# Linux-cpp-lisp/navigation-by-deja-vu

Measured on AMD Instinct MI355X. Metric: view-comparisons/sec (sensor x library x headings), higher is better.
Workload: dtype u8

## Files before the change

### navigation-by-deja-vu_amd/csrc/dejavu_hip.hip

```cpp
#include "dejavu_kernels.h"
#include "../../include/dejavu.h"

#include <algorithm>
#include <atomic>
#include <chrono>
#include <cmath>
#include <limits>
#include <cstdarg>
#include <cstddef>
#include <cstdint>
#include <cstdio>
#include <cstdlib>
#include <cstring>
#include <new>
#include <string>
#include <vector>

using namespace dv;

static_assert(sizeof(StepResultDev) == sizeof(dv_step_result) + sizeof(unsigned long long) &&
              offsetof(StepResultDev, check) == sizeof(dv_step_result), "device record = host record + check word");
static_assert(kMaxHeadings == DV_MAX_HEADINGS && kMaxHues == DV_MAX_HUE_PLANES, "header constants differ");
static_assert(kResSenseError == DV_RES_SENSE_ERROR, "header constants differ");

// ... 77 lines not shown
    uint4* d_tiles = nullptr;
    size_t tile_bytes = 0;

    unsigned char* d_raw_patches = nullptr;
    unsigned* d_prep = nullptr;
    PrepAcc* d_acc = nullptr;
    int acc_parity = 0;
    PrepBits pbits{};
    unsigned* d_one = nullptr;
    unsigned long long* d_bsum2 = nullptr;
    unsigned long long* d_bsum = nullptr;
    unsigned long long* d_ctmp = nullptr;
    int int_has_hs = 0, int_has_v = 0;
    int finish_vb_env = 0;
    int fenced_env = -1;
    int finish_fused = 1;
    unsigned* d_part = nullptr;
    unsigned long long* d_pmax = nullptr;
    int n_partial = 0;
    int nchunk = 1;
    int nchunk_cap = 1;
    int target_items = 0;
    int waves_per_cu = 0;
    int shape_env = 0;
    int force_shape = 0;
    int tuned_shape[4] = {0, 0, 0, 0};
    float tuned_us[4][6] = {};
    bool bits_ok = false;
    bool mixed = false;
    bool hs_bytes_pass = false;
    BitCfg bcfg{};
    uint4* d_btiles = nullptr;
    size_t btile_bytes = 0;
    uint4* d_coef = nullptr;
    bool coef_ready = false;
    bool prep_dwords_ready = false;
    int bits_env = 1;
    int mfma_tiles_env = 0, mfma_chunk_env = 0;
    const int* int_hsconst = nullptr;
    const int* int_vconst = nullptr;
    bool fuse_request = false;
    bool epilogue_fused = false;
    bool fp4_ok = false;
    int fp4_env = 1;
    uint4* d_coef4 = nullptr;
    uint4* d_ctiles = nullptr;
    size_t ctile_bytes = 0;
    int vcode_env = 0;
    int last_form = 0;
    int fuse_env = 1;
    int lc_env = 1;
    int ht_env = 2;
    int ring_env = 0;
    int mixed_env = 1;
    int tune_all_env = 0;
    int fail_alloc_env = 0;
    int lib_allocs = 0;
    int fused_nb = 0;
    int group_pad_kb = -1;
    int allow_signed = 1;
    double* d_fam = nullptr;
    double* d_scene = nullptr;
    StepState* d_state = nullptr;
    unsigned long long* d_cand = nullptr;
    double* d_cand_exact = nullptr;
    int result_slot = 0;
    struct PassSet {
        unsigned char* raw = nullptr; uint4* coef = nullptr; uint4* coef4 = nullptr; PrepAcc* acc = nullptr; int parity = 0;
        unsigned long long* bsum = nullptr; unsigned long long* ctmp = nullptr; StepState* state = nullptr;
        unsigned long long* cand = nullptr; double* cand_exact = nullptr;
        bool coef_ready = false, prep_dwords_ready = false, patches_sensed = false;
        int A = 0, APAD = 0, n_agents = 1, A_agent = 0, fused_nb = 0;
    };
    static constexpr int kExtraSets = 8;
    PassSet extra[kExtraSets];
    int n_extra = 0;
    int cur_set = 0;
    hipStream_t batch_stream = nullptr;
    hipStream_t batch_stream3 = nullptr;
    hipEvent_t ev_a = nullptr, ev_b = nullptr;
    bool defer_fold = false;
    int deferred_force = 0, deferred_seq = 0;
    int lc22_env = 1;
    int chain_order_env = -1;
    int chains_env = 2;
    StepResultDev* h_result = nullptr;
    StepResultDev* d_result = nullptr;
    double* d_record = nullptr;
    unsigned long long* d_keys = nullptr;
    double* h_scene = nullptr;
    int A = 0, APAD = 0;
    int n_agents = 1, A_agent = 0;
    bool step_pending = false;
    bool patches_sensed = false;
    int seq = 0;
    double* h_mbox = nullptr;
    double* d_mbox = nullptr;
    int mbox_rank = 0, mbox_world = 0, mbox_slots = 0;
    double* h_pub = nullptr;
    double* d_pub = nullptr;
    int64_t pub_cap = 0;
    unsigned long long pub_seq = 0;
    int spin_wait = 1;
    bool last_want_scene = false;
    double delta = 0.0;
    double wr_lo = 1.0, wr_hi = 0.0;
    AgentW* d_wts = nullptr;
    AgentW* h_wts = nullptr;
    int h_wts_cap = 0;
    bool wts_on = false;

    unsigned char* d_land = nullptr;
    SensorCfg sensor{};
    bool have_sensor = false;
    unsigned char* d_lut = nullptr;
    Pose* d_poses = nullptr;
    size_t poses_cap = 0;
    unsigned char* d_sense = nullptr;
    size_t sense_cap = 0;
    unsigned long long* d_sense_err = nullptr;
    std::vector<Pose> h_poses;

    double* d_path = nullptr;
    int64_t n_path = 0;
    unsigned char* d_cover = nullptr;
    unsigned char* d_cover_slots = nullptr;
    int n_cover_slots = 0;
    unsigned long long* d_minkeys = nullptr;
    unsigned long long* h_minkeys = nullptr;
    PathErrState* d_errstate = nullptr;
    PathErrOut* h_errout = nullptr;
    PathErrOut* d_errout = nullptr;
    unsigned long long err_enq = 0, err_deq = 0;
    int agent_pending = 0;
    bool err_on_main = false;

    hipEvent_t t0 = nullptr, t1 = nullptr;
    int profile = 0;
    long long profile_count = 0;
    std::vector<hipEvent_t> pev;
    size_t pev_used = 0;
};

static int fail(dv_ctx* c, int code, const char* fmt, ...) {
    char buf[512];
    va_list ap;
    va_start(ap, fmt);
    vsnprintf(buf, sizeof buf, fmt, ap);
    va_end(ap);
    if (c) c->err = buf; else g_create_error = buf;
    return code;
}

#define HIP_TRY(ctx, expr)                                                                      \
    do {                                                                                        \
        hipError_t e_ = (expr);                                                                 \
        if (e_ != hipSuccess)                                                                   \
            return fail(ctx, e_ == hipErrorOutOfMemory ? DV_ERR_OOM : DV_ERR_HIP, "%s: %s (%s:%d)", #expr, \
                        hipGetErrorString(e_), __FILE__, __LINE__);                             \
    } while (0)

static void use_set(dv_ctx* c, int which);
static void free_library(dv_ctx* c) {
    auto F = [](auto*& p) { if (p) { (void)hipFree(p); p = nullptr; } };
    use_set(c, 0);
    for (int j = 0; j < dv_ctx::kExtraSets; ++j) {
        dv_ctx::PassSet& a = c->extra[j];
        F(a.raw); F(a.coef); F(a.coef4); F(a.acc); F(a.bsum); F(a.ctmp); F(a.state); F(a.cand); F(a.cand_exact);
        a = dv_ctx::PassSet{};
    }
    c->n_extra = 0;
    F(c->d_tiles); F(c->d_raw_patches); F(c->d_prep); F(c->d_acc); F(c->d_one); F(c->d_fam); F(c->d_scene);
    F(c->d_part); F(c->d_pmax); F(c->d_record); F(c->d_keys); F(c->d_bsum); F(c->d_bsum2); F(c->d_ctmp);
    F(c->d_ftiles); F(c->d_fraw); F(c->d_fprep); F(c->d_fpart); F(c->d_fprep4); F(c->d_fvnorm); F(c->d_fpnorm); F(c->d_flower); F(c->d_fprepb);
    F(c->d_u8tiles); F(c->d_u8raw); F(c->d_u8prep); F(c->d_u8part); F(c->d_vnorm); F(c->d_pnorm);
    F(c->d_btiles); F(c->d_coef); F(c->d_coef4); F(c->d_ctiles); c->ctile_bytes = 0;
    c->pbits = PrepBits{};
    c->bits_ok = false; c->coef_ready = false; c->btile_bytes = 0;
    c->metric = 0;
    F(c->d_state); F(c->d_cand); F(c->d_cand_exact);
    if (c->h_result) { (void)hipHostFree(c->h_result); c->h_result = nullptr; c->d_result = nullptr; }
    if (c->h_scene) { (void)hipHostFree(c->h_scene); c->h_scene = nullptr; }
    c->have_lib = false;
    for (int i = 0; i < 4; ++i) c->tuned_shape[i] = 0;
    c->A = 0;
    c->step_pending = false;
}

extern "C" const char* dv_version(void) { return "dejavu-mi355x 0.1 (gfx950)"; }

extern "C" const char* dv_last_error(const dv_ctx* ctx) { return ctx ? ctx->err.c_str() : g_create_error.c_str(); }

extern "C" int dv_create(dv_ctx** out, int device_id) {
    if (!out) return fail(nullptr, DV_ERR_INVALID, "dv_create: out is NULL");
    *out = nullptr;
    int n = 0;
    HIP_TRY(nullptr, hipGetDeviceCount(&n));
    if (device_id < 0 || device_id >= n) return fail(nullptr, DV_ERR_INVALID, "dv_create: device %d of %d", device_id, n);
    HIP_TRY(nullptr, hipSetDevice(device_id));
    dv_ctx* c = new (std::nothrow) dv_ctx();
    if (!c) return fail(nullptr, DV_ERR_OOM, "dv_create: out of host memory");
    c->device = device_id;
    hipError_t e = hipStreamCreateWithFlags(&c->own_stream, hipStreamNonBlocking);
    if (e == hipSuccess) e = hipStreamCreateWithFlags(&c->aux_stream, hipStreamNonBlocking);
    if (e == hipSuccess) e = hipEventCreate(&c->t0);
    if (e == hipSuccess) e = hipEventCreate(&c->t1);
    if (e != hipSuccess) {
        fail(nullptr, DV_ERR_HIP, "dv_create: %s", hipGetErrorString(e));
        delete c;
        return DV_ERR_HIP;
    }
    c->stream = c->own_stream;
    auto env_int = [](const char* name, int& dst, int lo, int hi) {
        if (const char* t = getenv(name)) { const int v = atoi(t); if (v >= lo && v <= hi) dst = v; }
    };
    env_int("DEJAVU_TARGET_ITEMS", c->target_items, 1, 1 << 24);
    env_int("DEJAVU_WPC", c->waves_per_cu, 1, 32);
    env_int("DEJAVU_SHAPE", c->shape_env, 0, 6);
    env_int("DEJAVU_BITS", c->bits_env, 0, 2);
    env_int("DEJAVU_MFMA_TILES", c->mfma_tiles_env, 0, 2);
    env_int("DEJAVU_MFMA_CHUNK", c->mfma_chunk_env, 0, 32);
    env_int("DEJAVU_FINISH", c->finish_fused, 0, 2);
    env_int("DEJAVU_FENCED", c->fenced_env, 0, 1);
    env_int("DEJAVU_FINISH_VB", c->finish_vb_env, 0, 16);
    env_int("DEJAVU_FUSE", c->fuse_env, 0, 1);
    env_int("DEJAVU_FP4", c->fp4_env, 0, 1);
    env_int("DEJAVU_VCODE", c->vcode_env, 0, 1);
    env_int("DEJAVU_SIGNED", c->allow_signed, 0, 1);
    env_int("DEJAVU_GPAD", c->group_pad_kb, 0, 4096);
    env_int("DEJAVU_SPIN", c->spin_wait, 0, 1);
    env_int("DEJAVU_LC", c->lc_env, 0, 2);
    env_int("DEJAVU_HT", c->ht_env, 1, 2);
    env_int("DEJAVU_RING", c->ring_env, 0, 2);
    env_int("DEJAVU_MIXED", c->mixed_env, 0, 1);
    env_int("DEJAVU_TUNE_ALL", c->tune_all_env, 0, 1);
    env_int("DEJAVU_SSD_MFMA", c->ssd_mfma_env, 0, 3);
    env_int("DEJAVU_CHAINS", c->chains_env, 1, 3);
    env_int("DEJAVU_CHAIN_ORDER", c->chain_order_env, -1, 2);
    env_int("DEJAVU_LC22", c->lc22_env, 0, 1);
    env_int("DEJAVU_NT", c->nt_env, 0, 1);
    env_int("DEJAVU_TEST_FAIL_ALLOC", c->fail_alloc_env, 0, 64);
    *out = c;
    return DV_OK;
}

extern "C" void dv_destroy(dv_ctx* c) {
    if (!c) return;
    (void)hipSetDevice(c->device);
    (void)hipStreamSynchronize(c->stream);
    free_library(c);
    if (c->d_land) (void)hipFree(c->d_land);
    if (c->d_lut) (void)hipFree(c->d_lut);
    if (c->d_poses) (void)hipFree(c->d_poses);
    if (c->d_sense) (void)hipFree(c->d_sense);
    if (c->d_sense_err) (void)hipFree(c->d_sense_err);
    if (c->d_path) (void)hipFree(c->d_path);
    if (c->d_cover) (void)hipFree(c->d_cover);
    if (c->d_cover_slots) (void)hipFree(c->d_cover_slots);
    if (c->d_minkeys) (void)hipFree(c->d_minkeys);
    if (c->h_minkeys) (void)hipHostFree(c->h_minkeys);
    if (c->d_errstate) (void)hipFree(c->d_errstate);
    if (c->h_errout) (void)hipHostFree(c->h_errout);
    if (c->h_pub) (void)hipHostFree(c->h_pub);
    if (c->h_mbox) (void)hipHostUnregister(c->h_mbox);
    for (auto e : c->pev) (void)hipEventDestroy(e);
    if (c->t0) (void)hipEventDestroy(c->t0);
    if (c->t1) (void)hipEventDestroy(c->t1);
    if (c->aux_stream) { (void)hipStreamSynchronize(c->aux_stream); (void)hipStreamDestroy(c->aux_stream); }
    if (c->batch_stream) { (void)hipStreamSynchronize(c->batch_stream); (void)hipStreamDestroy(c->batch_stream); }
    if (c->batch_stream3) { (void)hipStreamSynchronize(c->batch_stream3); (void)hipStreamDestroy(c->batch_stream3); }
    if (c->d_wts) (void)hipFree(c->d_wts);
    if (c->h_wts) (void)hipHostFree(c->h_wts);
    if (c->ev_a) (void)hipEventDestroy(c->ev_a);
    if (c->ev_b) (void)hipEventDestroy(c->ev_b);
    if (c->own_stream) (void)hipStreamDestroy(c->own_stream);
    delete c;
}

extern "C" int dv_set_stream(dv_ctx* c, void* s) {
    if (!c) return DV_ERR_INVALID;
    HIP_TRY(c, hipStreamSynchronize(c->stream));
    c->stream = s ? (hipStream_t)s : c->own_stream;
    return DV_OK;
}

extern "C" int dv_set_exact(dv_ctx* c, int exact) {
    if (!c) return DV_ERR_INVALID;
    c->exact = exact ? 1 : 0;
    return DV_OK;
}

extern "C" int dv_set_mailbox(dv_ctx* c, void* host_base, int64_t bytes, int rank, int world) {
    if (!c) return DV_ERR_INVALID;
    HIP_TRY(c, hipSetDevice(c->device));
    HIP_TRY(c, hipStreamSynchronize(c->stream));
    if (c->h_mbox) { (void)hipHostUnregister(c->h_mbox); c->h_mbox = nullptr; c->d_mbox = nullptr; }
    if (!host_base) return DV_OK;
    const int64_t per_slot = (int64_t)world * kMboxEntry * (int64_t)sizeof(double);
    if (world < 1 || world > 64 || rank < 0 || rank >= world || bytes < per_slot || ((uintptr_t)host_base & 4095))
        return fail(c, DV_ERR_INVALID, "dv_set_mailbox: bad arguments");
    HIP_TRY(c, hipHostRegister(host_base, (size_t)bytes, hipHostRegisterMapped | hipHostRegisterPortable));
    c->h_mbox = (double*)host_base;
    HIP_TRY(c, hipHostGetDevicePointer((void**)&c->d_mbox, host_base, 0));
    c->mbox_rank = rank; c->mbox_world = world; c->mbox_slots = (int)(bytes / per_slot);
    return DV_OK;
}

extern "C" int dv_mailbox_post(dv_ctx* c, int slot, uint64_t seq) {
    if (!c) return DV_ERR_INVALID;
    if (!c->d_mbox || slot < 0 || slot >= c->mbox_slots) return fail(c, DV_ERR_STATE, "dv_mailbox_post: no mailbox or bad slot");
    if (!c->have_lib || c->A < 1) return fail(c, DV_ERR_STATE, "no library or no resident patches");
    HIP_TRY(c, hipSetDevice(c->device));
    double* entry = c->d_mbox + ((size_t)slot * c->mbox_world + c->mbox_rank) * kMboxEntry;
    hipLaunchKernelGGL(k_post, dim3(1), dim3(256), 0, c->stream, c->d_record, entry, 3 + 4 * c->A, (unsigned long long)seq);
    HIP_TRY(c, hipGetLastError());
    return DV_OK;
}

extern "C" int dv_mailbox_wait(dv_ctx* c, int slot, uint64_t seq, uint64_t rank_mask, double* records, int64_t stride,
                               int timeout_ms) {
    if (!c || !records) return DV_ERR_INVALID;
    if (!c->h_mbox || slot < 0 || slot >= c->mbox_slots || c->A < 1) return fail(c, DV_ERR_STATE, "dv_mailbox_wait: no mailbox or bad slot");
// ... 1482 lines not shown
    if (sh == 6) return c->bits_ok;
    const bool both_sums = !c->cfg.generic && c->cfg.nhs > 0 && c->cfg.hasv;
    return sh == 5 && both_sums;
}
static int shape_now(dv_ctx* c) {
    const int cls = apad_class(c->APAD);
    int s = c->force_shape ? c->force_shape : (c->shape_env ? c->shape_env : c->tuned_shape[cls]);
    if (!shape_valid(c, cls, s)) s = 1;
    return s;
}

template <int NHS, int HASV>
static void launch_tiles_apad(dv_ctx* c) {
    const int s = shape_now(c);
    if constexpr (NHS > 0 && HASV == 1) {
        if (s == 5) return launch_packed_apad<NHS>(c);
    }
    if (c->APAD == 8) {
        if (s == 2) launch_tiles_shape<NHS, HASV, 8, 8, 4, 1>(c);
        else launch_tiles_shape<NHS, HASV, 8, 8, 1, 1>(c);
    } else if (c->APAD == 16) {
        if (s == 2) launch_tiles_shape<NHS, HASV, 16, 16, 4, 1>(c);
        else if (s == 3) launch_tiles_shape<NHS, HASV, 8, 16, 1, 2>(c);
        else launch_tiles_shape<NHS, HASV, 16, 16, 1, 1>(c);
    } else if (c->APAD == 32) {
        if (s == 2) launch_tiles_shape<NHS, HASV, 32, 32, 4, 1>(c);
        else if (s == 3) launch_tiles_shape<NHS, HASV, 16, 32, 1, 2>(c);
        else launch_tiles_shape<NHS, HASV, 32, 32, 1, 1>(c);
    } else {
        if (s == 2) launch_tiles_shape<NHS, HASV, 32, 64, 4, 1>(c);
        else if (s == 3) launch_tiles_shape<NHS, HASV, 32, 64, 1, 2>(c);
        else if (s == 4) launch_tiles_shape<NHS, HASV, 16, 64, 1, 4>(c);
        else launch_tiles_shape<NHS, HASV, 32, 64, 1, 1>(c);
    }
}

template <int HAS_HS, int HASV, int AP, int ATOT>
static void launch_generic(dv_ctx* c) {
    static const int wpc = resident_waves_per_cu((const void*)k_sad_generic<HAS_HS, HASV, AP, ATOT>);
    dim3 block;
    const dim3 grid = scoring_grid(c, wpc, block);
    for (int a_off = 0; a_off < ATOT; a_off += AP)
        hipLaunchKernelGGL((k_sad_generic<HAS_HS, HASV, AP, ATOT>), grid, block, 0, c->stream, c->d_tiles, c->d_prep, c->d_part,
                           c->cfg, c->nchunk, a_off);
}

template <int HAS_HS, int HASV>
static void launch_generic_apad(dv_ctx* c) {
    if (c->APAD == 8) launch_generic<HAS_HS, HASV, 8, 8>(c);
    else if (c->APAD == 16) launch_generic<HAS_HS, HASV, 16, 16>(c);
    else if (c->APAD == 32) launch_generic<HAS_HS, HASV, 32, 32>(c);
    else launch_generic<HAS_HS, HASV, 32, 64>(c);
}

static const AgentW* wts_ptr(const dv_ctx* c) {
    return c->wts_on ? c->d_wts + (size_t)c->cur_set * kMaxHeadings : nullptr;
}

static FuseArgs fuse_args(const dv_ctx* c) {
    FuseArgs fz{};
    fz.wts = wts_ptr(c);
    fz.hsconst = c->d_acc[c->acc_parity].bhs;
    fz.vconst = c->d_acc[c->acc_parity].bv;
    fz.bsum = c->d_bsum;
    fz.ctmp = c->d_ctmp;
    fz.st = c->d_state;
    fz.A_real = c->A;
    fz.A_agent = c->A_agent;
    fz.delta = c->delta;
    return fz;
}

static long long item_groups(long long G32, int VW) {
    return (G32 + VW - 1) / VW;
}

template <int SK8, int RD8, int SK4, int RD4, int TILES, bool FUSE, int SKL, int RDL, bool LCODE, int HT>
static void launch_mfma_dual_f(dv_ctx* c, int nchunk, int has_hs) {
    static bool attr_set = false;
    const size_t lds8 = (size_t)RD8 * (SK8 * 8 + 8 * SK8 * TILES) * 1024;
    const size_t lds4 = (size_t)fp4_ring_bytes(SK4, TILES, RD4);
    size_t lds = lds8 > lds4 ? lds8 : lds4;
    if constexpr (SKL > 0) {
        constexpr int lcb = lc_ring_bytes<SKL, RDL>();
        static_assert(lcb + kFuseScratchBytes + (HT - 1) * 512 <= 160 * 1024, "LDS");
        if ((size_t)lcb > lds) lds = (size_t)lcb;
    }
    lds += FUSE ? (size_t)kFuseScratchBytes + (HT - 1) * 512 : 0;
    static_assert(fp4_ring_bytes(SK4, TILES, RD4) + kFuseScratchBytes <= 160 * 1024, "LDS");
    if (!attr_set) {
        (void)hipFuncSetAttribute((const void*)k_sad_mfma_dual<SK8, RD8, SK4, RD4, TILES, FUSE, SKL, RDL, LCODE, HT>, hipFuncAttributeMaxDynamicSharedMemorySize, (int)lds);
        attr_set = true;
    }
    const long long G32 = c->cfg.Fpad / 32;
    const long long n_gq = item_groups(G32, 8 * TILES / HT);
    const long long items = n_gq * nchunk;
    const unsigned grid = (unsigned)(items < 256 ? items : 256);
    const int nkt = c->bcfg.NK[0] + c->bcfg.NK[1];
    FuseArgs fz{};
    if (FUSE) { fz = fuse_args(c); fz.nb = (int)grid; }
    for (int a_off = 0; a_off < c->APAD; a_off += 32 * HT)
        hipLaunchKernelGGL((k_sad_mfma_dual<SK8, RD8, SK4, RD4, TILES, FUSE, SKL, RDL, LCODE, HT>), dim3(grid), dim3(512), lds, c->stream, c->d_btiles,
                           c->bcfg.vcode ? c->d_ctiles : c->d_btiles, c->d_coef + (size_t)(a_off / 32) * nkt * 512,
                           c->fp4_ok ? c->d_coef4 + (size_t)(a_off / 32) * nkt * 256 : nullptr, offlevel_word(c), reinterpret_cast<int*>(c->d_part),
                           c->cfg, c->bcfg, nchunk, c->APAD, a_off, has_hs, fz, (int)n_gq);
    if (FUSE) { c->epilogue_fused = true; c->fused_nb = (int)grid; }
}

template <int SK8, int RD8, int SK4, int RD4, int TILES, int SKL = 0, int RDL = 3, bool LCODE = false, int HT = 1>
static void launch_mfma_dual(dv_ctx* c, int nchunk, int has_hs) {
    if (c->fuse_request && nchunk == 1 && c->fuse_env) launch_mfma_dual_f<SK8, RD8, SK4, RD4, TILES, true, SKL, RDL, LCODE, HT>(c, nchunk, has_hs);
    else launch_mfma_dual_f<SK8, RD8, SK4, RD4, TILES, false, SKL, RDL, LCODE, HT>(c, nchunk, has_hs);
}

struct MfmaPlan { bool use_lc, two_tiles, lc22; int tiles, nchunk; };
static bool lc22_fits(const dv_ctx* c) {
    if (!c->lc22_env || !c->fp4_ok || c->bcfg.vcode || c->mixed) return false;
    for (int seg = 0; seg < 2; ++seg) {
        int w = 0;
        for (int bit = 1; bit < 4; ++bit) {
            const int wb = c->bcfg.wacc[seg][bit];
            if (wb && w && wb != w) return false;
            if (wb) w = wb;
        }
        if (seg == 0 && c->bcfg.wacc[0][0] && w && c->bcfg.wacc[0][0] != w) return false;
    }
    return (long long)c->bcfg.NK[0] * 256 <= 32767;
}
static MfmaPlan mfma_plan(dv_ctx* c, int apad, bool fuse_request) {
    MfmaPlan p{};
    const long long G32 = c->cfg.Fpad / 32;
    p.use_lc = c->lc_env != 0 && c->fp4_ok && !c->mfma_tiles_env;
    p.tiles = c->mfma_tiles_env ? c->mfma_tiles_env : (p.use_lc ? 1 : (G32 >= 16ll * 320 ? 2 : 1));
    if (p.tiles == 2 && !c->mfma_tiles_env) {
        static const bool spills[2] = {kernel_uses_scratch((const void*)k_sad_mfma_dual<1, 3, 2, 3, 2, false, 0, 3, false, 1>),
                                       kernel_uses_scratch((const void*)k_sad_mfma_dual<1, 3, 2, 3, 2, true, 0, 3, false, 1>)};
        const bool will_fuse = fuse_request && c->fuse_env && !c->mfma_chunk_env && item_groups(G32, 16) >= 160;
        if (spills[will_fuse ? 1 : 0]) p.tiles = 1;
    }
    p.two_tiles = p.use_lc && apad == 64 && c->ht_env == 2;
    p.lc22 = p.two_tiles && fuse_request && c->fuse_env && !c->mfma_chunk_env && lc22_fits(c) && item_groups(G32, 8) >= 160;
    const long long GQ = item_groups(G32, p.lc22 ? 8 : (p.two_tiles ? 4 : 8 * p.tiles));
    int nchunk = 1;
    if (c->mfma_chunk_env) {
        nchunk = c->mfma_chunk_env;
    } else if (GQ < 160) {
        nchunk = (int)((256 + GQ - 1) / GQ);
    }
    const int nk_min = c->bcfg.NK[1] > 0 ? (c->bcfg.NK[0] > 0 && c->bcfg.NK[0] < c->bcfg.NK[1] ? c->bcfg.NK[0] : c->bcfg.NK[1]) : c->bcfg.NK[0];
    while (nchunk > 1 && nk_min / nchunk < 4) --nchunk;
    if (nchunk > c->nchunk_cap) nchunk = c->nchunk_cap;
    if (nchunk < 1 || c->mixed) nchunk = 1;
    p.nchunk = nchunk;
    if (nchunk != 1) p.lc22 = false;
    return p;
}

template <int SKL, int RDL>
static void launch_lc22(dv_ctx* c, int has_hs) {
    static bool attr_set = false;
    size_t lds = (size_t)lc22_ring_bytes<SKL, RDL>() + kLc22ParkBytes;
    const size_t lds8 = (size_t)2 * (4 * 8 + 8 * 4) * 1024;
    if (lds8 > lds) lds = lds8;
    lds += (size_t)kFuseScratchBytes + 512;
    if (!attr_set) {
        (void)hipFuncSetAttribute((const void*)k_sad_lc22<SKL, RDL>, hipFuncAttributeMaxDynamicSharedMemorySize, (int)lds);
        attr_set = true;
    }
    const long long G32 = c->cfg.Fpad / 32;
    const long long n_gq = item_groups(G32, 8);
    const unsigned grid = (unsigned)(n_gq < 256 ? n_gq : 256);
    const int nkt = c->bcfg.NK[0] + c->bcfg.NK[1];
    FuseArgs fz = fuse_args(c);
    fz.nb = (int)grid;
    for (int a_off = 0; a_off < c->APAD; a_off += 64)
        hipLaunchKernelGGL((k_sad_lc22<SKL, RDL>), dim3(grid), dim3(512), lds, c->stream, c->d_btiles, c->d_coef + (size_t)(a_off / 32) * nkt * 512,
                           c->d_coef4 + (size_t)(a_off / 32) * nkt * 256, offlevel_word(c), c->cfg, c->bcfg, c->APAD, a_off, has_hs, fz, (int)n_gq);
    c->epilogue_fused = true;
    c->fused_nb = (int)grid;
}

static bool batch_pass_fuses(dv_ctx* c, int apad) {
    if (c->metric != 0 || c->exact || c->cfg.generic || !c->bits_ok || c->mixed || !c->fuse_env) return false;
    const int cls = apad_class(apad);
    const int shape = c->shape_env ? c->shape_env : c->tuned_shape[cls];
    if (shape != 6) return false;
    return mfma_plan(c, apad, true).nchunk == 1;
}

static void launch_mfma(dv_ctx* c, int has_hs) {
    const MfmaPlan plan = mfma_plan(c, c->APAD, c->fuse_request);
    const bool use_lc = plan.use_lc, two_tiles = plan.two_tiles;
    const int tiles = plan.tiles, nchunk = plan.nchunk, lc = c->lc_env;
    c->nchunk = nchunk;
    const int ring = c->ring_env;
    if (plan.lc22) launch_lc22<2, 3>(c, has_hs);
    else if (two_tiles && c->bcfg.vcode) launch_mfma_dual<4, 2, 2, 4, 1, 4, 3, true, 2>(c, nchunk, has_hs);
    else if (two_tiles) launch_mfma_dual<4, 2, 2, 4, 1, 4, 3, false, 2>(c, nchunk, has_hs);
    else if (use_lc && c->bcfg.vcode) launch_mfma_dual<4, 2, 2, 4, 1, 4, 3, true>(c, nchunk, has_hs);
    else if (use_lc && lc == 2) launch_mfma_dual<4, 2, 2, 4, 1, 2, 5>(c, nchunk, has_hs);
    else if (use_lc) launch_mfma_dual<4, 2, 2, 4, 1, 4, 3>(c, nchunk, has_hs);
    else if (tiles == 2) launch_mfma_dual<1, 3, 2, 3, 2>(c, nchunk, has_hs);
    else if (ring == 1) launch_mfma_dual<4, 2, 2, 6, 1>(c, nchunk, has_hs);
    else if (ring == 2) launch_mfma_dual<4, 2, 4, 3, 1>(c, nchunk, has_hs);
    else launch_mfma_dual<4, 2, 2, 4, 1>(c, nchunk, has_hs);
}

static int launch_int_scoring(dv_ctx* c, hipEvent_t after_tiles, int* n_partial, bool with_combine = true) {
    const LibCfg& g = c->cfg;
    int has_hs_sum, has_v_sum = g.hasv;
    c->int_hsconst = c->d_acc[c->acc_parity].hs;
    c->int_vconst = nullptr;
    c->epilogue_fused = false;
    c->last_form = 0;
    if (needs_prep_dwords(c)) { const int rc = ensure_prep_dwords(c); if (rc) return rc; }
    if (!g.generic && shape_now(c) == 6) {
        if (!c->coef_ready) { const int rc = enqueue_bit_prep(c, true); if (rc) return rc; }
        has_hs_sum = g.nhs > 0 ? 1 : 0;
        if (c->mixed) {
            c->fuse_request = false;
            launch_mfma(c, has_hs_sum);
            HIP_TRY(c, hipGetLastError());
            c->hs_bytes_pass = true;
            const int keep = c->force_shape;
            c->force_shape = c->APAD >= 16 ? 2 : 1;
            switch (g.nhs) {
                case 1: launch_tiles_apad<1, 0>(c); break;
                case 2: launch_tiles_apad<2, 0>(c); break;
                case 3: launch_tiles_apad<3, 0>(c); break;
                default: launch_tiles_apad<4, 0>(c); break;
            }
            c->force_shape = keep;
            c->hs_bytes_pass = false;
            c->nchunk = 1;
        } else
        launch_mfma(c, has_hs_sum);
        c->last_form = DV_FORM_MATRIX_CORES | (c->fp4_ok ? DV_FORM_FP4 : 0) | (c->epilogue_fused ? DV_FORM_FUSED_FINISH : 0);
        c->int_hsconst = c->mixed ? c->d_acc[c->acc_parity].hs : c->d_acc[c->acc_parity].bhs;
        c->int_vconst = c->d_acc[c->acc_parity].bv;
    } else if (g.generic) {
        has_hs_sum = 1;
        if (g.hasv) launch_generic_apad<1, 1>(c); else launch_generic_apad<1, 0>(c);
    } else {
        has_hs_sum = g.nhs > 0 ? 1 : 0;
        switch (g.nhs * 2 + g.hasv) {
            case 1: launch_tiles_apad<0, 1>(c); break;
            case 2: launch_tiles_apad<1, 0>(c); break;
            case 3: launch_tiles_apad<1, 1>(c); break;
            case 4: launch_tiles_apad<2, 0>(c); break;
            case 5: launch_tiles_apad<2, 1>(c); break;
            case 6: launch_tiles_apad<3, 0>(c); break;
            case 7: launch_tiles_apad<3, 1>(c); break;
            case 8: launch_tiles_apad<4, 0>(c); break;
            case 9: launch_tiles_apad<4, 1>(c); break;
            default: return fail(c, DV_ERR_STATE, "unsupported plane configuration nhs=%d hasv=%d", g.nhs, g.hasv);
        }
    }
    HIP_TRY(c, hipGetLastError());
    if (after_tiles) HIP_TRY(c, hipEventRecord(after_tiles, c->stream));
    c->int_has_hs = has_hs_sum;
    c->int_has_v = has_v_sum;
    if (c->epilogue_fused) return DV_OK;
    if (!with_combine) return DV_OK;
    *n_partial = (int)((g.Fpad + 1023) / 1024);
    hipLaunchKernelGGL(k_combine, dim3((unsigned)*n_partial, (unsigned)c->A), dim3(256), 0, c->stream, c->d_part, c->int_hsconst,
                       c->int_vconst, c->d_fam, c->d_pmax, c->d_state, c->cfg, c->nchunk, c->APAD, has_hs_sum, has_v_sum, c->n_agents, wts_ptr(c),
                       c->A_agent);
    HIP_TRY(c, hipGetLastError());
    return DV_OK;
}

static int tune_workgroup_shape(dv_ctx* c) {
    hipEvent_t ev[2];
    HIP_TRY(c, hipEventCreate(&ev[0]));
    HIP_TRY(c, hipEventCreate(&ev[1]));
    const int cls = apad_class(c->APAD);
    for (int i = 0; i < 6; ++i) c->tuned_us[cls][i] = 0.f;
    float best = 0.f;
    bool timed_any = false;
    int rc = DV_OK, pick = 1, np = 0;
    const bool fuse_request = c->fuse_request;
    c->fuse_request = false;
// ... 874 lines not shown
```

### navigation-by-deja-vu_amd/csrc/dejavu_kernels.h

```cpp
#pragma once
#include <hip/hip_runtime.h>
#include <stdint.h>
#include <type_traits>

#pragma clang fp contract(off)

namespace dv {

#ifdef DEJAVU_STAMPS
#ifdef DEJAVU_EXP_FIN
#define DV_EXP_FIN_ON 1
#else
#define DV_EXP_FIN_ON 0
#endif
__device__ unsigned long long g_dv_stamps[256 * 8];
#define DV_STAMP(i) do { if (threadIdx.x == 0) { g_dv_stamps[(blockIdx.x & 255) * 8 + (i)] = __builtin_amdgcn_s_memrealtime(); \
    if (((i) == 1 || (i) == 2) && !DV_EXP_FIN_ON) g_dv_stamps[(blockIdx.x & 255) * 8 + 5 + (i)] = __builtin_amdgcn_s_memtime(); } } while (0)
#else
#define DV_STAMP(i) do { } while (0)
#endif

constexpr int kMaxHeadings = 64;
constexpr int kMaxHues = 4;
constexpr int kCandCap = 4096;
// ... 3533 lines not shown
                            if constexpr (!code_stage) {
                                x[0] = xl[k & 1][t].x; x[1] = xl[k & 1][t].y; x[2] = xl[k & 1][t].z; x[3] = xl[k & 1][t].w;
                            } else {
                                if constexpr (k == 0) { x[0] = xl[0][t].x; x[1] = xl[0][t].y; x[2] = xl[0][t].z; }
                                else if constexpr (k == 1) { x[0] = xl[0][t].w; x[1] = xl[1][t].x; x[2] = xl[1][t].y; }
                                else if constexpr (k == 2) { x[0] = xl[1][t].z; x[1] = xl[1][t].w; x[2] = xc2[t].x; }
                                else { x[0] = xc2[t].y; x[1] = xc2[t].z; x[2] = xc2[t].w; }
                                x[3] = ((x[0] >> 3) & 0x11111111u) | ((x[1] >> 2) & 0x22222222u) | ((x[2] >> 1) & 0x44444444u);
                            }
                        };
                        if constexpr (HT == 1) {
#pragma unroll
                            for (int t = 0; t < TL; ++t) {
                                unsigned x[4];
                                load_x(t, x);
#pragma unroll
                                for (int s = 0; s < 4; ++s) {
                                    unsigned o[4];
                                    operand(x, s, o);
                                    mfma(t, s, o[0], o[1], o[2], o[3]);
                                }
                            }
                        } else {
                            if constexpr (h == 0) {
                                unsigned x[4];
                                load_x(0, x);
#pragma unroll
                                for (int s = 0; s < 4; ++s) operand(x, s, bo[s]);
                            }
#pragma unroll
                            for (int s = 0; s < 4; ++s) mfma(h, s, bo[s][0], bo[s][1], bo[s][2], bo[s][3]);
                        }
                    });
                    cslot = nslot;
                }
            };
            const int nst0 = has_hs_sum ? (NK0 / SK < nst ? NK0 / SK : nst) : 0;
            const int hs_end = (has_hs_sum && !(c.hasv && b.NK[1] > 0)) ? nst : nst0;
            run_stages(0, hs_end, IntC<0>{});
            if (hs_end > 0 && hs_end < nst) {
                flush(tot_hs, b.wacc[0], false);
                if constexpr (!FUSE) store_sums(tot_hs, 0);
#pragma unroll
                for (int u = 0; u < 2; ++u)
#pragma unroll
                    for (int s = 0; s < 4; ++s)
#pragma unroll
                        for (int r = 0; r < 16; ++r) acc[u][s][r] = 0.f;
            }
            if constexpr (CODE) run_stages(hs_end, nst, IntC<1>{});
            else run_stages(hs_end, nst, IntC<0>{});
            if (hs_end < nst) flush(tot_v, b.wacc[1], codev);
            else flush(tot_hs, b.wacc[0], false);
            if constexpr (!FUSE) {
                if (has_hs_sum && !(hs_end > 0 && hs_end < nst)) store_sums(tot_hs, 0);
                if (c.hasv) store_sums(tot_v, 1);
            }
        }
        if (j == 0) DV_STAMP(2);
        if constexpr (FUSE) {
            if (j == 0) DV_STAMP(3);
            if constexpr (HT == 1) {
                auto of_hs = [&](int t, int r) -> int { return tot_hs[t][r]; };
                auto of_v = [&](int t, int r) -> int { return tot_v[t][r]; };
                fused_finish<TL, NW, true>(of_hs, of_v, gidx, live, scratch0, c, fz, a_off, has_hs_sum, j, lane, wave, (int)(j & 1), NC, hconst[0]);
            } else {
#pragma unroll
                for (int h = 0; h < HT; ++h) {
                    auto of_hs = [&](int, int r) -> int { return tot_hs[h][r]; };
                    auto of_v = [&](int, int r) -> int { return tot_v[h][r]; };
                    if (a_off + 32 * h < fz.A_real)
                        fused_finish<TL, NW, true>(of_hs, of_v, gidx, live, scratch0, c, fz, a_off + 32 * h, has_hs_sum, j, lane, wave, nfin++ & 1, NC,
                                             hconst[h], scratch0 + kFuseBlk + h * 64);
                }
            }
            if (j == 0) DV_STAMP(4);
        }
    }
    }
    if constexpr (FUSE) {
#pragma unroll
        for (int h = 0; h < HT; ++h)
            if (a_off + 32 * h < fz.A_real) fused_block_end(scratch0 + h * 64, fz, c, a_off + 32 * h);
    }
    DV_STAMP(5);
}

template <int SK, int RD>
constexpr int lc22_ring_bytes() { return RD * SK * 16 * 1024; }
constexpr int kLc22ParkBytes = 4 * 64 * 64 * 2;

template <int SK, int RD>
__device__ __forceinline__ void
sad_lc22_fp4(const uint4* __restrict__ ftiles, const uint4* __restrict__ coef4, const LibCfg& c, const BitCfg& b, int apad_total, int a_off,
             int has_hs_sum, const FuseArgs& fz, int n_gq) {
    extern __shared__ uint4 lds_ring[];
    constexpr int HT = 2, TL = 2;
    constexpr int NW = 8, NC = 4, NL = 4;
    constexpr int KCOEF = 4 * HT, KLIB = NC * TL;
    constexpr int COEF_ROWS = SK * KCOEF, ROWS = SK * (KCOEF + KLIB);
    constexpr int SLOTB = ROWS * 1024;
    constexpr int PER = ROWS / NL;
    constexpr int RING = RD * SLOTB;
    constexpr int NU = SK * HT;
    static_assert(PER == SK * (HT + TL) && PER * (RD - 1) < 64 && RD >= 3, "ring shape");
    static_assert(RING + kLc22ParkBytes + kFuseScratchBytes + 512 <= 160 * 1024, "LDS");
    const int lane = threadIdx.x & 63;
    const int wave = __builtin_amdgcn_readfirstlane(threadIdx.x >> 6);
    const bool loader = wave >= NC;
    const long long G32 = c.Fpad / 32, GQ = n_gq;
    const int NKT = b.NK[0] + b.NK[1];
    const int nst = (NKT + SK - 1) / SK;
    const int NK0 = b.NK[0];
    const long long gbytes = (long long)b.GS * 1024;
    const long long pass16 = (long long)NKT * 256;
    const unsigned lds_base = (unsigned)(unsigned long long)(lds_ptr_t)lds_ring;
    unsigned char* lds_bytes = reinterpret_cast<unsigned char*>(lds_ring);
    short* park = reinterpret_cast<short*>(lds_bytes + RING) + (wave & 3) * (64 * 64);
    unsigned long long* scratch0 = reinterpret_cast<unsigned long long*>(lds_bytes + RING + kLc22ParkBytes);
    const unsigned char* lib_bytes = reinterpret_cast<const unsigned char*>(ftiles);
    DV_STAMP(0);
#pragma unroll
    for (int h = 0; h < HT; ++h) fused_block_begin(scratch0 + h * 64, h == 0);
    const long long n_mine = GQ > (long long)blockIdx.x ? (GQ - blockIdx.x + gridDim.x - 1) / gridDim.x : 0;

    if (loader) {
        const int lw = wave - NC;
        long long li = 0;
        int lst = 0, lslot = 0;
        const unsigned char* lp[TL];
        bool llive[TL];
#pragma unroll
        for (int t = 0; t < TL; ++t) { lp[t] = lib_bytes; llive[t] = false; }
        auto loader_item = [&]() {
#pragma unroll
            for (int t = 0; t < TL; ++t) llive[t] = false;
            if (li < n_mine) {
                const long long item = blockIdx.x + li * gridDim.x;
                const long long g0 = (item * G32) / GQ, g1 = ((item + 1) * G32) / GQ;
#pragma unroll
                for (int t = 0; t < TL; ++t) {
                    const long long g = g0 + lw + 4 * t;
                    llive[t] = g < g1;
                    lp[t] = lib_bytes + (llive[t] ? g : g0) * gbytes + lane * 16;
                }
            }
        };
        const bool nt_rows = b.nt != 0;
        auto issue_stage = [&]() {
            const unsigned slot = lds_base + (unsigned)lslot * (unsigned)SLOTB;
            const int kb = lst * SK;
            const uint4* hot = coef4 + lw * 64 + lane;
#pragma unroll
            for (int i = 0; i < SK * HT; ++i) {
                const int kk = i / HT, h = i % HT;
                int k = kb + kk;
                k = k < NKT ? k : NKT - 1;
                const unsigned dst = __builtin_amdgcn_readfirstlane(slot + (unsigned)((kk * KCOEF + h * 4 + lw) * 1024));
#ifdef DEJAVU_EXP22
                if (DEJAVU_EXP22 & 4) continue;
#endif
                lds_dma_16(li < n_mine ? coef4 + h * pass16 + ((long long)k * 4 + lw) * 64 + lane : hot, dst);
            }
#pragma unroll
            for (int i = 0; i < SK * TL; ++i) {
#ifdef DEJAVU_EXP22
// ... 158 lines not shown
                        for (int t = 0; t < TL; ++t) lds_tie(xl[0][t]);
                    }
#pragma unroll
                    for (int t = 0; t < TL; ++t)
#pragma unroll
                        for (int h = 0; h < HT; ++h)
#pragma unroll
                            for (int r = 0; r < 16; ++r)
                                park[((t * HT + h) * 16 + r) * 64 + lane] = (short)((int)acc[t][h][0][r] + (int)acc[t][h][1][r]);
                    if (hs_end < nst) clear();
                }
                if (hs_end < nst) {
                    run_stages(hs_end, nst);
                    const int w0 = w_of(1, 0), w1 = w_of(1, 1);
#pragma unroll
                    for (int t = 0; t < TL; ++t)
#pragma unroll
                        for (int h = 0; h < HT; ++h)
#pragma unroll
                            for (int r = 0; r < 16; ++r) tot_v[t][h][r] = __mul24(w0, (int)acc[t][h][0][r]) + __mul24(w1, (int)acc[t][h][1][r]);
                } else {
#pragma unroll
                    for (int t = 0; t < TL; ++t)
#pragma unroll
                        for (int h = 0; h < HT; ++h)
#pragma unroll
                            for (int r = 0; r < 16; ++r) tot_v[t][h][r] = 0;
                }
            }
            if (j == 0) DV_STAMP(2);
#pragma unroll
            for (int h = 0; h < HT; ++h) {
                if (j == 0) DV_STAMP(3 + h);
                auto of_hs = [&](int t, int r) -> int { return __mul24(whs, (int)park[((t * HT + h) * 16 + r) * 64 + lane]); };
                auto of_v = [&](int t, int r) -> int { return tot_v[t][h][r]; };
#ifdef DEJAVU_EXP22
                if (DEJAVU_EXP22 & 32) {
                    if (a_off + 32 * h < fz.A_real) {
                        if (of_hs(0, 0) + of_v(1, 15) == 0x7fffffff) park[lane] = 1;
                        fused_finish_idle();
                    }
                    continue;
                }
#endif
                if (a_off + 32 * h < fz.A_real)
                    fused_finish<TL, NW, true>(of_hs, of_v, gidx, live, scratch0, c, fz, a_off + 32 * h, has_hs_sum, j, lane, wave, nfin++ & 1, NC,
                                               hconst[h], scratch0 + kFuseBlk + h * 64);
            }
            if (j == 0) DV_STAMP(5);
        }
    }
#pragma unroll
    for (int h = 0; h < HT; ++h)
        if (a_off + 32 * h < fz.A_real) fused_block_end(scratch0 + h * 64, fz, c, a_off + 32 * h);
    (void)apad_total;
}

template <int SKL, int RDL>
__global__ void __launch_bounds__(512, 2)
k_sad_lc22(const uint4* __restrict__ btiles, const uint4* __restrict__ coef, const uint4* __restrict__ coef4, const unsigned* __restrict__ offlevel,
           LibCfg c, BitCfg b, int apad_total, int a_off, int has_hs_sum, FuseArgs fz, int n_gq) {
    const bool fp4 = __builtin_amdgcn_readfirstlane(*offlevel) == 0u;
    if (fp4) {
        sad_lc22_fp4<SKL, RDL>(btiles, coef4, c, b, apad_total, a_off, has_hs_sum, fz, n_gq);
        return;
    }
    const int NKT = b.NK[0] + b.NK[1];
#pragma unroll 1
    for (int h = 0; h < 2; ++h) {
        if (h > 0 && a_off + 32 * h >= apad_total) break;
        sad_ring_i8<4, 1, 2, true>(btiles, coef + (long long)h * NKT * 512, nullptr, c, b, 1, apad_total, a_off + 32 * h, has_hs_sum, fz, n_gq);
    }
}

template <int SK8, int RD8, int SK4, int RD4, int TILES, bool FUSE, int SKL, int RDL, bool LCODE, int HT>
__global__ void __launch_bounds__(512, 2)
k_sad_mfma_dual(const uint4* __restrict__ btiles, const uint4* __restrict__ ftiles, const uint4* __restrict__ coef, const uint4* __restrict__ coef4,
                const unsigned* __restrict__ offlevel, int* __restrict__ part, LibCfg c, BitCfg b, int nchunk, int apad_total, int a_off,
                int has_hs_sum, FuseArgs fz, int n_gq) {
    const bool fp4 = __builtin_amdgcn_readfirstlane(*offlevel) == 0u;
    if constexpr (SKL > 0) {
        static_assert(TILES == 1, "the loader / consumer body cuts the library into ranges of 8 / HT view groups; the other bodies must agree");
        if (fp4 && nchunk == 1) {
            sad_lc_fp4<SKL, RDL, FUSE, LCODE, HT>(ftiles, coef4, part, c, b, apad_total, a_off, has_hs_sum, fz, n_gq);
            return;
        }
    }
    const int NKT = b.NK[0] + b.NK[1];
#pragma unroll 1
    for (int h = 0; h < HT; ++h) {
        if (h > 0 && a_off + 32 * h >= apad_total) break;
        if (fp4) sad_ring_fp4<SK4, TILES, RD4, FUSE>(btiles, coef4 + (long long)h * NKT * 256, part, c, b, nchunk, apad_total, a_off + 32 * h, has_hs_sum, fz, n_gq);
        else sad_ring_i8<SK8, TILES, RD8, FUSE>(btiles, coef + (long long)h * NKT * 512, part, c, b, nchunk, apad_total, a_off + 32 * h, has_hs_sum, fz, n_gq);
    }
}


constexpr int kStreamRows = 16;
__global__ void __launch_bounds__(512)
k_stream_read(const uint4* __restrict__ src, long long n16, unsigned* __restrict__ sink) {
    extern __shared__ uint4 lds_stream[];
    const int lane = threadIdx.x & 63;
    const int wave = __builtin_amdgcn_readfirstlane(threadIdx.x >> 6);
    const unsigned base = (unsigned)(unsigned long long)(lds_ptr_t)lds_stream + (unsigned)wave * (unsigned)kStreamRows * 1024u;
    const long long rows = n16 / 64;
    const long long stride = (long long)gridDim.x * 8;
    long long row = (long long)blockIdx.x * 8 + wave;
    for (; row + (kStreamRows - 1) * stride < rows; row += kStreamRows * stride) {
#pragma unroll
        for (int i = 0; i < kStreamRows; ++i) lds_dma_16_nt(src + (row + i * stride) * 64 + lane, __builtin_amdgcn_readfirstlane(base + (unsigned)i * 1024u));
        wait_vmcnt_le<0>();
    }
    for (; row < rows; row += stride) {
        lds_dma_16_nt(src + row * 64 + lane, __builtin_amdgcn_readfirstlane(base));
        wait_vmcnt_le<0>();
    }
    if (lds_stream[threadIdx.x].x == 0x9E3779B9u && lds_stream[threadIdx.x].y == 0x12345u) sink[0] = 1;
}

}
```

Before: 15.81 billion.

## Stream library tiles straight to registers in a new fp4 LC kernel variant

Adds a loader/consumer fp4 MFMA body where only the sensor coefficients are staged through the LDS ring by loader waves. Consumer waves load library rows directly from global memory into registers with nontemporal loads, one stage ahead, and expand the bit planes in-register. The goal is to cut LDS capacity and traffic for library tiles and let a deeper stage (SK=8) fit. It is selected by default when lc==1, nchunk==1 and the weight pattern fits. The risks are register pressure and exposed global latency on the consumer waves.

```diff
diff --git a/navigation-by-deja-vu_amd/csrc/dejavu_hip.hip b/navigation-by-deja-vu_amd/csrc/dejavu_hip.hip
--- a/navigation-by-deja-vu_amd/csrc/dejavu_hip.hip
+++ b/navigation-by-deja-vu_amd/csrc/dejavu_hip.hip
@@ -183,6 +183,7 @@
     bool defer_fold = false;
     int deferred_force = 0, deferred_seq = 0;
     int lc22_env = 1;
+    int lreg_env = 1;
     int chain_order_env = -1;
     int chains_env = 2;
     StepResultDev* h_result = nullptr;
@@ -339,6 +340,7 @@
     env_int("DEJAVU_CHAINS", c->chains_env, 1, 3);
     env_int("DEJAVU_CHAIN_ORDER", c->chain_order_env, -1, 2);
     env_int("DEJAVU_LC22", c->lc22_env, 0, 1);
+    env_int("DEJAVU_LIBREG", c->lreg_env, 0, 1);
     env_int("DEJAVU_NT", c->nt_env, 0, 1);
     env_int("DEJAVU_TEST_FAIL_ALLOC", c->fail_alloc_env, 0, 64);
     *out = c;
@@ -1987,7 +1989,7 @@
     const size_t lds4 = (size_t)fp4_ring_bytes(SK4, TILES, RD4);
     size_t lds = lds8 > lds4 ? lds8 : lds4;
     if constexpr (SKL > 0) {
-        constexpr int lcb = lc_ring_bytes<SKL, RDL>();
+        constexpr int lcb = SKL == kLregStage ? lreg_ring_bytes<SKL, RDL>() : lc_ring_bytes<SKL, RDL>();
         static_assert(lcb + kFuseScratchBytes + (HT - 1) * 512 <= 160 * 1024, "LDS");
         if ((size_t)lcb > lds) lds = (size_t)lcb;
     }
@@ -2032,6 +2034,18 @@
     }
     return (long long)c->bcfg.NK[0] * 256 <= 32767;
 }
+static bool lreg_fits(const dv_ctx* c) {
+    if (!c->lreg_env || !c->fp4_ok || c->bcfg.vcode || c->mixed) return false;
+    for (int seg = 0; seg < 2; ++seg) {
+        int w = 0;
+        for (int bit = 1; bit < 4; ++bit) {
+            const int wb = c->bcfg.wacc[seg][bit];
+            if (wb && w && wb != w) return false;
+            if (wb) w = wb;
+        }
+    }
+    return c->bcfg.NK[0] % kLregStage == 0;
+}
 static MfmaPlan mfma_plan(dv_ctx* c, int apad, bool fuse_request) {
     MfmaPlan p{};
     const long long G32 = c->cfg.Fpad / 32;
@@ -2103,6 +2117,7 @@
     else if (two_tiles && c->bcfg.vcode) launch_mfma_dual<4, 2, 2, 4, 1, 4, 3, true, 2>(c, nchunk, has_hs);
     else if (two_tiles) launch_mfma_dual<4, 2, 2, 4, 1, 4, 3, false, 2>(c, nchunk, has_hs);
     else if (use_lc && c->bcfg.vcode) launch_mfma_dual<4, 2, 2, 4, 1, 4, 3, true>(c, nchunk, has_hs);
+    else if (use_lc && lc == 1 && nchunk == 1 && lreg_fits(c)) launch_mfma_dual<4, 2, 2, 4, 1, kLregStage, 3>(c, nchunk, has_hs);
     else if (use_lc && lc == 2) launch_mfma_dual<4, 2, 2, 4, 1, 2, 5>(c, nchunk, has_hs);
     else if (use_lc) launch_mfma_dual<4, 2, 2, 4, 1, 4, 3>(c, nchunk, has_hs);
     else if (tiles == 2) launch_mfma_dual<1, 3, 2, 3, 2>(c, nchunk, has_hs);
diff --git a/navigation-by-deja-vu_amd/csrc/dejavu_kernels.h b/navigation-by-deja-vu_amd/csrc/dejavu_kernels.h
--- a/navigation-by-deja-vu_amd/csrc/dejavu_kernels.h
+++ b/navigation-by-deja-vu_amd/csrc/dejavu_kernels.h
@@ -3639,6 +3639,249 @@
 #pragma unroll
         for (int h = 0; h < HT; ++h)
             if (a_off + 32 * h < fz.A_real) fused_block_end(scratch0 + h * 64, fz, c, a_off + 32 * h);
+    }
+    DV_STAMP(5);
+}
+
+constexpr int kLregStage = 8;
+template <int SK, int RD>
+constexpr int lreg_ring_bytes() { return RD * SK * 4 * 1024; }
+
+template <int SK, int RD, bool FUSE>
+__device__ __forceinline__ void
+sad_lc_fp4_lreg(const uint4* __restrict__ btiles, const uint4* __restrict__ coef4, int* __restrict__ part, const LibCfg& c, const BitCfg& b,
+                int apad_total, int a_off, int has_hs_sum, const FuseArgs& fz, int n_gq) {
+    extern __shared__ uint4 lds_ring[];
+    constexpr int TL = 2;
+    constexpr int NW = 8, NC = 4;
+    constexpr int KCOEF = 4;
+    constexpr int SLOTB = SK * KCOEF * 1024;
+    constexpr int PER = SK;
+    constexpr int RING = RD * SLOTB;
+    static_assert(PER * (RD - 1) < 64 && SK % 2 == 0 && RD >= 3, "ring shape");
+    const int lane = threadIdx.x & 63;
+    const int wave = __builtin_amdgcn_readfirstlane(threadIdx.x >> 6);
+    const bool loader = wave >= NC;
+    const long long G32 = c.Fpad / 32, GQ = n_gq;
+    const int NKT = b.NK[0] + b.NK[1];
+    const int nst = (NKT + SK - 1) / SK;
+    const int NK0 = b.NK[0];
+    const long long gbytes = (long long)b.GS * 1024;
+    const unsigned lds_base = (unsigned)(unsigned long long)(lds_ptr_t)lds_ring;
+    unsigned long long* scratch0 = reinterpret_cast<unsigned long long*>(reinterpret_cast<unsigned char*>(lds_ring) + RING);
+    const unsigned char* lib_bytes = reinterpret_cast<const unsigned char*>(btiles);
+    DV_STAMP(0);
+    if constexpr (FUSE) fused_block_begin(scratch0, true);
+    const long long n_mine = GQ > (long long)blockIdx.x ? (GQ - blockIdx.x + gridDim.x - 1) / gridDim.x : 0;
+
+    if (loader) {
+        const int lw = wave - NC;
+        long long li = 0;
+        int lst = 0, lslot = 0;
+        auto issue_stage = [&]() {
+            const unsigned slot = lds_base + (unsigned)lslot * (unsigned)SLOTB;
+            const int kb = lst * SK;
+            const uint4* hot = coef4 + lw * 64 + lane;
+#pragma unroll
+            for (int kk = 0; kk < SK; ++kk) {
+                int k = kb + kk;
+                k = k < NKT ? k : NKT - 1;
+                const unsigned dst = __builtin_amdgcn_readfirstlane(slot + (unsigned)((kk * KCOEF + lw) * 1024));
+                lds_dma_16(li < n_mine ? coef4 + ((long long)k * 4 + lw) * 64 + lane : hot, dst);
+            }
+            lslot = lslot + 1 == RD ? 0 : lslot + 1;
+            if (++lst == nst) { lst = 0; ++li; }
+        };
+#pragma unroll
+        for (int r = 0; r < RD - 1; ++r) issue_stage();
+        for (long long j = 0; j < n_mine; ++j) {
+            for (int st = 0; st < nst; ++st) {
+                wait_vmcnt_le<PER * (RD - 2)>();
+                __builtin_amdgcn_s_barrier();
+                issue_stage();
+            }
+            if constexpr (FUSE) fused_finish_idle();
+        }
+        wait_vmcnt_le<0>();
+    } else {
+        int cslot = 0;
+        int hconst[2] = {0, 0};
+        if (FUSE) {
+            const int a = a_off + (lane & 31), ac = a < fz.A_real ? a : fz.A_real - 1;
+            hconst[0] = acc_sum(fz.hsconst, ac);
+            hconst[1] = fz.vconst ? acc_sum(fz.vconst, ac) : 0;
+        }
+        auto w_of = [&](int seg, int cls) -> int {
+            if (cls == 0) return b.wacc[seg][0];
+            const int w1 = b.wacc[seg][1], w2 = b.wacc[seg][2], w3 = b.wacc[seg][3];
+            return w1 ? w1 : (w2 ? w2 : w3);
+        };
+        long long lj = 0;
+        int lkb = 0;
+        const unsigned char* cp[TL] = {lib_bytes, lib_bytes};
+        auto cursor_item = [&]() {
+            const long long item = blockIdx.x + (lj < n_mine ? lj : 0) * gridDim.x;
+            const long long g0 = (item * G32) / GQ, g1 = ((item + 1) * G32) / GQ;
+#pragma unroll
+            for (int t = 0; t < TL; ++t) {
+                const long long g = g0 + wave * TL + t;
+                cp[t] = lib_bytes + (g < g1 ? g : g0) * gbytes + lane * 16;
+            }
+        };
+        v4u_t xr[SK][TL];
+        auto load_row = [&](int kk) {
+            int k = lkb + kk;
+            k = k < NKT ? k : NKT - 1;
+#pragma unroll
+            for (int t = 0; t < TL; ++t) xr[kk][t] = __builtin_nontemporal_load(reinterpret_cast<const v4u_t*>(cp[t] + (long long)k * 1024));
+        };
+        auto cursor_next = [&]() {
+            lkb += SK;
+            if (lkb >= nst * SK) { lkb = 0; ++lj; cursor_item(); }
+        };
+        if (n_mine > 0) {
+            cursor_item();
+#pragma unroll
+            for (int kk = 0; kk < SK; ++kk) load_row(kk);
+            cursor_next();
+        }
+        for (long long j = 0; j < n_mine; ++j) {
+            const long long item = blockIdx.x + j * gridDim.x;
+            const long long g0 = (item * G32) / GQ, g1 = ((item + 1) * G32) / GQ;
+            long long gidx[TL];
+            bool live[TL];
+#pragma unroll
+            for (int t = 0; t < TL; ++t) {
+                const long long g = g0 + wave * TL + t;
+                live[t] = g < g1;
+                gidx[t] = live[t] ? g : g0;
+            }
+            int tot_hs[TL][16], tot_v[TL][16];
+#pragma unroll
+            for (int t = 0; t < TL; ++t)
+#pragma unroll
+                for (int r = 0; r < 16; ++r) { tot_hs[t][r] = 0; tot_v[t][r] = 0; }
+            auto store_sums = [&](const int (&tot)[TL][16], int seg) {
+                const int rows = (apad_total - a_off) < 32 ? (apad_total - a_off) : 32;
+#pragma unroll
+                for (int t = 0; t < TL; ++t) {
+                    if (!live[t]) continue;
+                    const int type_row = seg ? has_hs_sum : 0;
+                    int* dst = part + ((long long)type_row * apad_total + a_off) * c.Fpad + gidx[t] * 32 + (lane & 31);
+                    int half = lane >> 5;
+                    asm volatile("" : "+v"(half));
+#pragma unroll
+                    for (int r = 0; r < 16; ++r) {
+                        const int m = (r & 3) + 8 * (r >> 2) + 4 * half;
+                        if (m < rows) dst[(long long)m * c.Fpad] = tot[t][r];
+                    }
+                }
+            };
+            {
+                v16f_t acc[TL][2];
+                auto clear = [&]() {
+#pragma unroll
+                    for (int t = 0; t < TL; ++t)
+#pragma unroll
+                        for (int cl = 0; cl < 2; ++cl)
+#pragma unroll
+                            for (int r = 0; r < 16; ++r) acc[t][cl][r] = 0.f;
+                };
+                auto flush = [&](int (&dst)[TL][16], int seg) {
+                    const int w0 = w_of(seg, 0), w1 = w_of(seg, 1);
+#pragma unroll
+                    for (int t = 0; t < TL; ++t)
+#pragma unroll
+                        for (int r = 0; r < 16; ++r) dst[t][r] = __mul24(w0, (int)acc[t][0][r]) + __mul24(w1, (int)acc[t][1][r]);
+                };
+                clear();
+                v4u_t a[2][4];
+                auto fetch = [&](int slot_i, auto kc) {
+                    constexpr int kk = decltype(kc)::value;
+                    const unsigned sad = lds_base + (unsigned)slot_i * (unsigned)SLOTB + (unsigned)lane * 16u;
+                    static_for<4>([&](auto sc) { constexpr int s_ = decltype(sc)::value; lds_read16<(kk * KCOEF + s_) * 1024>(a[kk & 1][s_], sad); });
+                };
+                __builtin_amdgcn_s_barrier();
+                if (j == 0) DV_STAMP(1);
+                fetch(cslot, IntC<0>{});
+                auto run_stages = [&](int s0, int s1) {
+                    for (int st = s0; st < s1; ++st) {
+                        const int kb = st * SK;
+                        const int nslot = cslot + 1 == RD ? 0 : cslot + 1;
+                        static_for<SK>([&](auto kc) {
+                            constexpr int kk = decltype(kc)::value;
+                            if constexpr (kk + 1 < SK) {
+                                fetch(cslot, IntC<kk + 1>{});
+                                lds_wait<4>();
+                            } else {
+                                lds_wait<0>();
+                                if (st + 1 < nst) {
+                                    __builtin_amdgcn_s_barrier();
+                                    fetch(nslot, IntC<0>{});
+                                }
+                            }
+#pragma unroll
+                            for (int s = 0; s < 4; ++s) lds_tie(a[kk & 1][s]);
+                            const unsigned m = kb + kk < NKT ? 0x22222222u : 0u;
+                            unsigned bo[TL][4][4];
+#pragma unroll
+                            for (int t = 0; t < TL; ++t) lds_tie(xr[kk][t]);
+#pragma unroll
+                            for (int t = 0; t < TL; ++t) {
+                                const unsigned x[4] = {xr[kk][t].x, xr[kk][t].y, xr[kk][t].z, xr[kk][t].w};
+#pragma unroll
+                                for (int d = 0; d < 4; ++d) {
+                                    bo[t][0][d] = (x[d] << 1) & m;
+                                    bo[t][1][d] = x[d] & m;
+                                    bo[t][2][d] = (x[d] >> 1) & m;
+                                    bo[t][3][d] = (x[d] >> 2) & m;
+                                }
+                            }
+                            load_row(kk);
+#pragma unroll
+                            for (int s = 0; s < 4; ++s) {
+                                const v4u_t& av = a[kk & 1][s];
+                                const v8i_t ao = v8i_t{(int)av.x, (int)av.y, (int)av.z, (int)av.w, 0, 0, 0, 0};
+#pragma unroll
+                                for (int t = 0; t < TL; ++t) {
+                                    const v8i_t bv = v8i_t{(int)bo[t][s][0], (int)bo[t][s][1], (int)bo[t][s][2], (int)bo[t][s][3], 0, 0, 0, 0};
+                                    if constexpr (FUSE) acc[t][s ? 1 : 0] = __builtin_amdgcn_mfma_scale_f32_32x32x64_f8f6f4(bv, ao, acc[t][s ? 1 : 0], 4, 4, 0, 0, 0, 0);
+                                    else acc[t][s ? 1 : 0] = __builtin_amdgcn_mfma_scale_f32_32x32x64_f8f6f4(ao, bv, acc[t][s ? 1 : 0], 4, 4, 0, 0, 0, 0);
+                                }
+                            }
+                        });
+                        cursor_next();
+                        cslot = nslot;
+                    }
+                };
+                const int nst0 = has_hs_sum ? (NK0 / SK < nst ? NK0 / SK : nst) : 0;
+                const int hs_end = (has_hs_sum && !(c.hasv && b.NK[1] > 0)) ? nst : nst0;
+                run_stages(0, hs_end);
+                if (hs_end > 0 && hs_end < nst) {
+                    flush(tot_hs, 0);
+                    if constexpr (!FUSE) store_sums(tot_hs, 0);
+                    clear();
+                }
+                run_stages(hs_end, nst);
+                if (hs_end < nst) flush(tot_v, 1);
+                else flush(tot_hs, 0);
+                if constexpr (!FUSE) {
+                    if (has_hs_sum && !(hs_end > 0 && hs_end < nst)) store_sums(tot_hs, 0);
+                    if (c.hasv) store_sums(tot_v, 1);
+                }
+            }
+            if (j == 0) DV_STAMP(2);
+            if constexpr (FUSE) {
+                if (j == 0) DV_STAMP(3);
+                auto of_hs = [&](int t, int r) -> int { return tot_hs[t][r]; };
+                auto of_v = [&](int t, int r) -> int { return tot_v[t][r]; };
+                fused_finish<TL, NW, true>(of_hs, of_v, gidx, live, scratch0, c, fz, a_off, has_hs_sum, j, lane, wave, (int)(j & 1), NC, hconst);
+                if (j == 0) DV_STAMP(4);
+            }
+        }
+    }
+    if constexpr (FUSE) {
+        if (a_off < fz.A_real) fused_block_end(scratch0, fz, c, a_off);
     }
     DV_STAMP(5);
 }
@@ -3963,7 +4206,12 @@
     if constexpr (SKL > 0) {
         static_assert(TILES == 1, "the loader / consumer body cuts the library into ranges of 8 / HT view groups; the other bodies must agree");
         if (fp4 && nchunk == 1) {
-            sad_lc_fp4<SKL, RDL, FUSE, LCODE, HT>(ftiles, coef4, part, c, b, apad_total, a_off, has_hs_sum, fz, n_gq);
+            if constexpr (SKL == kLregStage) {
+                static_assert(HT == 1 && !LCODE, "sad_lc_fp4_lreg: one heading tile, thermometer rows");
+                sad_lc_fp4_lreg<SKL, RDL, FUSE>(btiles, coef4, part, c, b, apad_total, a_off, has_hs_sum, fz, n_gq);
+            } else {
+                sad_lc_fp4<SKL, RDL, FUSE, LCODE, HT>(ftiles, coef4, part, c, b, apad_total, a_off, has_hs_sum, fz, n_gq);
+            }
             return;
         }
     }
```

Measured after the change: 16.27 billion (median of 6 runs). +2.9%, better.
